# NJUVISION/PCGCv1

Measured on AMD Instinct MI355X. Metric: 64³ cubes/sec encode+decode (hyper/a6b3); bpp & D1-PSNR vs reference, higher is better.
Workload: dtype f32; 1 GPU; synthetic longdress_vox10-like cloud (seed 1300, 1024^3): 828225 points -> 205 cubes of 64^3, --mode=hyper --cube_size=64 --min_num=64, the hyper/a6b3 checkpoint trained with this repository's train_hyper step on seeded synthetic surfaces (checkpoints/hyper/a6.00b3.00, tools/train_ckpt.py; the cloud was held out), compress_hyper + decompress_hyper incl. host range coding; cubes_per_rank=205, stream_crc32=2267905730

## Files before the change

include/pcgc.h:

```cpp
#ifndef PCGC_H_
#define PCGC_H_

#include <stddef.h>
#include <stdint.h>

#ifdef __cplusplus
extern "C" {
#endif

typedef void* pcgc_stream_t;

int pcgc_version(void);
const char* pcgc_last_error(void);

int pcgc_conv3d_fwd(const float* x, const float* kernel, const float* bias, float* y,
                    int B, int D, int Cin, int Cout, int ksize, int stride,
                    int transposed, int relu, int algo, pcgc_stream_t stream);

size_t pcgc_vrn_workspace_bytes(int B, int D, int C);
int pcgc_vrn_fwd(const float* x, const float* const* params, float* out, int B, int D, int C,
                 void* workspace, size_t workspace_bytes, pcgc_stream_t stream);

enum {
  PCGC_NET_ANALYSIS = 0,
// ... 6 lines not shown
int pcgc_net_param_count(int kind);
int pcgc_net_create(int kind, const float* const* params, int n_params,
                    pcgc_stream_t stream, pcgc_net** out);
void pcgc_net_destroy(pcgc_net* net);
int pcgc_net_set_algo(pcgc_net* net, int algo);
int pcgc_rowocc(const float* x, unsigned long long* rowocc, int B, pcgc_stream_t stream);
int pcgc_net_set_skip_counter(pcgc_net* net, unsigned* device_counter);
int pcgc_net_set_profiling(pcgc_net* net, int on);
int pcgc_net_profile_report(pcgc_net* net, char* buf, size_t cap, size_t* needed);
size_t pcgc_net_workspace_bytes(const pcgc_net* net, int B, int D);
int pcgc_net_forward(const pcgc_net* net, const float* x, float* out0, float* out1,
                     int B, int D, float scale_lower_bound, void* workspace,
                     size_t workspace_bytes, pcgc_stream_t stream);


int pcgc_repro_eval(int fn, const float* x, float* y, int64_t n, pcgc_stream_t stream);

int pcgc_round_minmax(const float* x, float* q, int32_t* seg_min, int32_t* seg_max,
                      int64_t n, int64_t seg_len, pcgc_stream_t stream);
int pcgc_round_minmax_i16(const float* x, int16_t* q, int32_t* seg_min, int32_t* seg_max,
                          int64_t n, int64_t seg_len, pcgc_stream_t stream);
int pcgc_symbols_to_values(const int16_t* sym, int offset, float* out, int64_t n, pcgc_stream_t stream);
int pcgc_symbols_to_values_seg(const int16_t* sym, const float* seg_offset, float* out, int64_t n, int64_t seg_len,
                               pcgc_stream_t stream);

int pcgc_laplace_likelihood(const float* y, const float* loc, const float* scale,
                            const float* noise, float* values, float* likelihood,
                            int64_t n, float likelihood_bound, pcgc_stream_t stream);

int pcgc_laplace_cdf(const float* loc, const float* scale, const int32_t* seg_min,
                     const int32_t* seg_max, int64_t rows, int64_t seg_rows, int ncols,
                     float likelihood_bound, const float* symbols, uint16_t* cdf_lower,
                     uint32_t* lohi, pcgc_stream_t stream);

int pcgc_factorized_likelihood(const float* z, const float* params, const float* noise,
                               float* values, float* likelihood, int64_t n, int C,
                               float likelihood_bound, pcgc_stream_t stream);
int pcgc_factorized_pmf(const float* params, int C, int min_v, int max_v,
                        float likelihood_bound, float* pmf, pcgc_stream_t stream);

int pcgc_topk_threshold(const float* x, const int32_t* k_per_cube, int B, int64_t vox,
                        int use_fixed, float fixed_thres, float* thresholds,
                        uint8_t* mask, void* workspace, size_t workspace_bytes,
                        pcgc_stream_t stream);
size_t pcgc_topk_workspace_bytes(int B, int64_t vox);

int pcgc_bce_sums(const float* pred, const float* label, int64_t n, double* sums4,
                  void* workspace, size_t workspace_bytes, pcgc_stream_t stream);
size_t pcgc_bce_workspace_bytes(int64_t n);

size_t pcgc_classify_workspace_bytes(void);
int pcgc_classify_sums(const float* pred, const float* label, int64_t n, float th, double* sums3,
                       void* workspace, size_t workspace_bytes, pcgc_stream_t stream);
int pcgc_confusion_matrix(const float* pred, const float* label, int64_t n, float th, float* tp,
                          float* fp, float* fn, pcgc_stream_t stream);

size_t pcgc_focal_workspace_bytes(void);
int pcgc_focal_loss(const float* y_pred, const float* y_true, int64_t n, float gamma, float alpha, double* loss,
                    void* workspace, size_t workspace_bytes, pcgc_stream_t stream);
int pcgc_focal_loss_bwd(const float* y_pred, const float* y_true, int64_t n, float gamma, float alpha,
                        float grad_scale, float* dy_pred, pcgc_stream_t stream);

size_t pcgc_d1_workspace_bytes(int res);
int pcgc_d1_mse(const int32_t* pa, int64_t na, const int32_t* pb, int64_t nb, int res, double* out2,
                void* workspace, size_t workspace_bytes, pcgc_stream_t stream);

// ... 261 lines not shown
int pcgc_laplace_likelihood_bwd_dev(const float* values, const float* loc, const float* scale, double num, double mul,
                                    const double* count, float likelihood_bound, float* dvalues, float* dloc,
                                    float* dscale, int64_t n, pcgc_stream_t stream);
int pcgc_factorized_likelihood_bwd_dev(const float* values, const float* params, double num, double mul,
                                       const double* count, float likelihood_bound, float* dvalues, float* dparams,
                                       int64_t n, int C, void* workspace, size_t workspace_bytes, pcgc_stream_t stream);
size_t pcgc_sum_log_workspace_bytes(void);
int pcgc_sum_log(const float* p, int64_t n, double* out, void* workspace, size_t workspace_bytes,
                 pcgc_stream_t stream);
size_t pcgc_train_loss_sums_workspace_bytes(int64_t n);
int pcgc_train_loss_sums(const float* pred, const float* label, int64_t n, const float* lik_y, int64_t n_y,
                         const float* lik_z, int64_t n_z, double* sums4, double* logs2, void* workspace,
                         size_t workspace_bytes, pcgc_stream_t stream);
int pcgc_adam_step(float* param, const float* grad, float* m, float* v, int64_t n, float lr_t, float beta1,
                   float beta2, float epsilon, pcgc_stream_t stream);
int pcgc_adam_step_guarded(float* param, const float* grad, float* m, float* v, int64_t n, float lr_t, float beta1,
                           float beta2, float epsilon, const double* bce_sums4, pcgc_stream_t stream);

const char* pcgc_host_last_error(void);

int pcgc_pmf_to_quantized_cdf(const float* pmf, int64_t rows, int n, int precision, int32_t* cdf);
int pcgc_range_encode(const int16_t* data, int64_t rows, int cols, const int32_t* cdf, int n,
                      int broadcast_rows, int precision, uint8_t* out, int64_t cap, int64_t* out_len);
int pcgc_range_encode_values(const void* data, int elem_bytes, int64_t rows, int cols, int offset, const int32_t* cdf, int n,
                             int broadcast_rows, int precision, uint8_t* out, int64_t cap, int64_t* out_len);
int pcgc_range_decode(const uint8_t* str, int64_t len, int64_t rows, int cols, const int32_t* cdf,
                      int n, int broadcast_rows, int precision, int16_t* out);
int pcgc_range_decode_progress(const uint8_t* str, int64_t len, int64_t rows, int cols, const int32_t* cdf,
                               int n, int broadcast_rows, int precision, int16_t* out, int64_t* progress);

int pcgc_range_encode_lohi_batch(const uint32_t* lohi, int n_streams, int64_t sym_per_stream,
                                 int precision, uint8_t* out, int64_t cap_per_stream,
                                 int64_t* out_lens, int n_threads);
int pcgc_range_decode_u16_batch(const uint8_t* strings, const int64_t* offsets, const int64_t* lens,
                                int n_streams, int64_t sym_per_stream, const uint16_t* cdf_lower,
                                int ncols, const int32_t* n_sym, int precision, int16_t* out,
                                int n_threads);

int pcgc_partition(const int32_t* points, int64_t n, int cube_size, int min_num, int64_t* n_cubes,
                   int64_t* cube_positions, int64_t* sorted_positions, int32_t* cube_of_point);

int pcgc_parse_ply_points(const char* text, int64_t len, int32_t* out, int64_t cap, int64_t* n_points, int n_threads);

int pcgc_format_points_int(const int64_t* pts, int64_t n, char* out, int64_t cap, int64_t* out_len);

int pcgc_parse_ply_columns(const char* text, int64_t len, const int32_t* columns, int k, int64_t max_rows, double* out,
                           int64_t cap, int64_t* n_rows, int n_threads);

int pcgc_format_points_colors_int(const int64_t* pts, const uint8_t* colors, int64_t n, char* out, int64_t cap,
                                  int64_t* out_len);

int pcgc_parse_mesh(const char* text, int64_t len, int format, double* vertices, int64_t vcap, int32_t* triangles,
                    int64_t tcap, int64_t* n_vertices, int64_t* n_triangles);
int pcgc_mesh_area_cdf(const double* vertices, int64_t n_vertices, const int32_t* triangles, int64_t n_triangles, double* cdf);

uint32_t pcgc_crc32c(uint32_t crc_in, const void* data, int64_t n);

int pcgc_host_repro_eval(int fn, const float* x, float* y, int64_t n);

#ifdef __cplusplus
}
#endif
#endif
```

pcgcv1_amd/_lib.py:

```python
import ctypes
import os


_HERE = os.path.dirname(os.path.abspath(__file__))
_LIBDIR = os.path.join(_HERE, "lib")

c_int, c_i64, c_f32, c_vp, c_sz = ctypes.c_int, ctypes.c_int64, ctypes.c_float, ctypes.c_void_p, ctypes.c_size_t

HIP_API = {
    "pcgc_version": (c_int, []),
    "pcgc_last_error": (ctypes.c_char_p, []),
    "pcgc_conv3d_fwd": (c_int, [c_vp, c_vp, c_vp, c_vp, c_int, c_int, c_int, c_int, c_int, c_int, c_int, c_int, c_int, c_vp]),
    "pcgc_vrn_workspace_bytes": (c_sz, [c_int, c_int, c_int]),
    "pcgc_vrn_fwd": (c_int, [c_vp, c_vp, c_vp, c_int, c_int, c_int, c_vp, c_sz, c_vp]),
    "pcgc_net_param_count": (c_int, [c_int]),
    "pcgc_net_create": (c_int, [c_int, c_vp, c_int, c_vp, c_vp]),
    "pcgc_net_destroy": (None, [c_vp]),
    "pcgc_net_set_algo": (c_int, [c_vp, c_int]),
    "pcgc_net_set_skip_counter": (c_int, [c_vp, c_vp]),
    "pcgc_rowocc": (c_int, [c_vp, c_vp, c_int, c_vp]),
    "pcgc_net_set_profiling": (c_int, [c_vp, c_int]),
    "pcgc_net_profile_report": (c_int, [c_vp, c_vp, c_sz, c_vp]),
    "pcgc_net_workspace_bytes": (c_sz, [c_vp, c_int, c_int]),
    "pcgc_net_forward": (c_int, [c_vp, c_vp, c_vp, c_vp, c_int, c_int, c_f32, c_vp, c_sz, c_vp]),
    "pcgc_repro_eval": (c_int, [c_int, c_vp, c_vp, c_i64, c_vp]),
    "pcgc_round_minmax": (c_int, [c_vp, c_vp, c_vp, c_vp, c_i64, c_i64, c_vp]),
    "pcgc_round_minmax_i16": (c_int, [c_vp, c_vp, c_vp, c_vp, c_i64, c_i64, c_vp]),
    "pcgc_symbols_to_values": (c_int, [c_vp, c_int, c_vp, c_i64, c_vp]),
    "pcgc_symbols_to_values_seg": (c_int, [c_vp, c_vp, c_vp, c_i64, c_i64, c_vp]),
    "pcgc_laplace_likelihood": (c_int, [c_vp, c_vp, c_vp, c_vp, c_vp, c_vp, c_i64, c_f32, c_vp]),
    "pcgc_laplace_cdf": (c_int, [c_vp, c_vp, c_vp, c_vp, c_i64, c_i64, c_int, c_f32, c_vp, c_vp, c_vp, c_vp]),
    "pcgc_factorized_likelihood": (c_int, [c_vp, c_vp, c_vp, c_vp, c_vp, c_i64, c_int, c_f32, c_vp]),
    "pcgc_factorized_pmf": (c_int, [c_vp, c_int, c_int, c_int, c_f32, c_vp, c_vp]),
    "pcgc_topk_threshold": (c_int, [c_vp, c_vp, c_int, c_i64, c_int, c_f32, c_vp, c_vp, c_vp, c_sz, c_vp]),
    "pcgc_topk_workspace_bytes": (c_sz, [c_int, c_i64]),
    "pcgc_bce_sums": (c_int, [c_vp, c_vp, c_i64, c_vp, c_vp, c_sz, c_vp]),
    "pcgc_bce_workspace_bytes": (c_sz, [c_i64]),
    "pcgc_classify_workspace_bytes": (c_sz, []),
    "pcgc_classify_sums": (c_int, [c_vp, c_vp, c_i64, c_f32, c_vp, c_vp, c_sz, c_vp]),
    "pcgc_confusion_matrix": (c_int, [c_vp, c_vp, c_i64, c_f32, c_vp, c_vp, c_vp, c_vp]),
    "pcgc_focal_workspace_bytes": (c_sz, []),
    "pcgc_focal_loss": (c_int, [c_vp, c_vp, c_i64, c_f32, c_f32, c_vp, c_vp, c_sz, c_vp]),
    "pcgc_focal_loss_bwd": (c_int, [c_vp, c_vp, c_i64, c_f32, c_f32, c_f32, c_vp, c_vp]),
    "pcgc_voxelize": (c_int, [c_vp, c_i64, c_int, c_vp, c_int, c_vp]),
    "pcgc_voxelize_points": (c_int, [c_vp, c_vp, c_i64, c_int, c_int, c_int, c_vp, c_vp]),
    "pcgc_pointnums_count": (c_int, [c_vp, c_vp, c_vp, c_int, c_int, c_vp, c_vp, c_vp, c_vp]),
    "pcgc_pointnums_curves_workspace_bytes": (c_sz, [c_i64, c_i64]),
    "pcgc_pointnums_curves": (c_int, [c_vp, c_vp, c_vp, c_int, c_int, c_vp, c_vp, c_vp, c_i64, c_i64, c_vp, c_int, c_vp, c_int,
                                      c_vp, c_vp, c_vp, c_vp, c_sz, c_vp]),
    "pcgc_pointnums_normals_workspace_bytes": (c_sz, [c_i64]),
    "pcgc_pointnums_normals": (c_int, [c_vp, c_vp, c_i64, c_vp, c_i64, c_vp, c_vp, c_sz, c_vp]),
    "pcgc_pointnums_curves_d2_workspace_bytes": (c_sz, [c_i64, c_i64]),
    "pcgc_pointnums_curves_d2": (c_int, [c_vp, c_vp, c_vp, c_vp, c_int, c_int, c_vp, c_vp, c_vp, c_i64, c_i64, c_vp, c_int, c_vp,
                                         c_int, c_vp, c_vp, c_vp, c_vp, c_sz, c_vp]),
    "pcgc_pointnums_sweep_workspace_bytes": (c_sz, [c_int, c_int]),
    "pcgc_pointnums_sweep": (c_int, [c_vp, c_vp, c_vp, c_vp, c_int, c_int, c_vp, c_int, c_vp, c_vp, c_vp, c_sz, c_vp]),
    "pcgc_mesh_sample": (c_int, [c_vp, c_i64, c_vp, c_i64, c_vp, c_i64, ctypes.c_uint64, c_vp, c_vp, c_vp]),
    "pcgc_mesh_voxelize_workspace_bytes": (c_sz, [c_int]),
    "pcgc_mesh_voxelize": (c_int, [c_vp, c_i64, c_int, c_vp, c_i64, c_vp, c_vp, c_sz, c_vp]),
    "pcgc_normals_table_size": (c_int, [ctypes.c_double]),
    "pcgc_normals_workspace_bytes": (c_sz, [c_int, c_i64, ctypes.c_double]),
    "pcgc_estimate_normals": (c_int, [c_vp, c_i64, c_int, ctypes.c_double, c_int, c_vp, c_vp, c_vp, c_vp, c_sz, c_vp]),
    "pcgc_ingest_bounds": (c_int, [c_vp, c_i64, c_vp, c_vp, c_vp]),
    "pcgc_ingest_quantize": (c_int, [c_vp, c_i64, c_vp, ctypes.c_double, c_int, c_vp, c_vp, c_vp]),
# ... 94 lines not shown
    "pcgc_train_conv_fwd": (c_int, [c_vp, c_int, c_vp, c_vp, c_vp, c_int, c_int, c_int, c_vp]),
    "pcgc_train_conv_bwd_data": (c_int, [c_vp, c_int, c_vp, c_vp, c_vp, c_vp, c_int, c_int, c_vp]),
    "pcgc_train_conv_bwd_weight": (c_int, [c_vp, c_int, c_vp, c_vp, c_int, c_int, c_vp]),
    "pcgc_train_conv_bwd_weight_pair": (c_int, [c_vp, c_int, c_int, c_vp, c_vp, c_vp, c_int, c_int, c_vp]),
    "pcgc_train_conv_fwd_pair": (c_int, [c_vp, c_int, c_int, c_vp, c_vp, c_vp, c_vp, c_vp, c_vp, c_int, c_int, c_int, c_int, c_vp]),
    "pcgc_train_conv_bwd_data_pair": (c_int, [c_vp, c_int, c_int, c_vp, c_vp, c_vp, c_vp, c_vp, c_vp, c_int, c_int, c_vp]),
    "pcgc_train_conv_bwd_data_chain": (c_int, [c_vp, c_int, c_int, c_vp, c_vp, c_vp, c_vp, c_int, c_int, c_vp]),
    "pcgc_train_conv_fwd_merge": (c_int, [c_vp, c_int, c_vp, c_vp, c_vp, c_int, c_vp, c_vp, c_vp, c_int, c_int, c_int, c_vp]),
    "pcgc_train_plan_finish_weights": (c_int, [c_vp, c_vp]),
    "pcgc_train_plan_defer_small": (c_int, [c_vp, c_int]),
    "pcgc_abs_max": (c_int, [c_vp, c_f32, c_vp, c_vp, c_i64, c_vp]),
    "pcgc_laplace_likelihood_bwd": (c_int, [c_vp, c_vp, c_vp, c_f32, c_f32, c_vp, c_vp, c_vp, c_i64, c_vp]),
    "pcgc_factorized_bwd_workspace_bytes": (c_sz, [c_int]),
    "pcgc_factorized_likelihood_bwd": (c_int, [c_vp, c_vp, c_f32, c_f32, c_vp, c_vp, c_i64, c_int, c_vp, c_sz, c_vp]),
    "pcgc_bce_bwd": (c_int, [c_vp, c_vp, c_f32, c_f32, c_vp, c_i64, c_vp]),
    "pcgc_bce_bwd_dev": (c_int, [c_vp, c_vp, c_vp, ctypes.c_double, ctypes.c_double, c_vp, c_i64, c_vp]),
    "pcgc_laplace_likelihood_bwd_dev": (c_int, [c_vp, c_vp, c_vp, ctypes.c_double, ctypes.c_double, c_vp, c_f32, c_vp, c_vp, c_vp, c_i64, c_vp]),
    "pcgc_factorized_likelihood_bwd_dev": (c_int, [c_vp, c_vp, ctypes.c_double, ctypes.c_double, c_vp, c_f32, c_vp, c_vp, c_i64, c_int, c_vp, c_sz, c_vp]),
    "pcgc_sum_log_workspace_bytes": (c_sz, []),
    "pcgc_sum_log": (c_int, [c_vp, c_i64, c_vp, c_vp, c_sz, c_vp]),
    "pcgc_train_loss_sums_workspace_bytes": (c_sz, [c_i64]),
    "pcgc_train_loss_sums": (c_int, [c_vp, c_vp, c_i64, c_vp, c_i64, c_vp, c_i64, c_vp, c_vp, c_vp, c_sz, c_vp]),
    "pcgc_adam_step": (c_int, [c_vp, c_vp, c_vp, c_vp, c_i64, c_f32, c_f32, c_f32, c_f32, c_vp]),
    "pcgc_adam_step_guarded": (c_int, [c_vp, c_vp, c_vp, c_vp, c_i64, c_f32, c_f32, c_f32, c_f32, c_vp, c_vp]),
}
HOST_API = {
    "pcgc_host_last_error": (ctypes.c_char_p, []),
    "pcgc_pmf_to_quantized_cdf": (c_int, [c_vp, c_i64, c_int, c_int, c_vp]),
    "pcgc_range_encode": (c_int, [c_vp, c_i64, c_int, c_vp, c_int, c_int, c_int, c_vp, c_i64, c_vp]),
    "pcgc_range_encode_values": (c_int, [c_vp, c_int, c_i64, c_int, c_int, c_vp, c_int, c_int, c_int, c_vp, c_i64, c_vp]),
    "pcgc_range_decode": (c_int, [c_vp, c_i64, c_i64, c_int, c_vp, c_int, c_int, c_int, c_vp]),
    "pcgc_range_decode_progress": (c_int, [c_vp, c_i64, c_i64, c_int, c_vp, c_int, c_int, c_int, c_vp, c_vp]),
    "pcgc_range_encode_lohi_batch": (c_int, [c_vp, c_int, c_i64, c_int, c_vp, c_i64, c_vp, c_int]),
    "pcgc_range_decode_u16_batch": (c_int, [c_vp, c_vp, c_vp, c_int, c_i64, c_vp, c_int, c_vp, c_int, c_vp, c_int]),
    "pcgc_partition": (c_int, [c_vp, c_i64, c_int, c_int, c_vp, c_vp, c_vp, c_vp]),
    "pcgc_crc32c": (ctypes.c_uint32, [ctypes.c_uint32, c_vp, c_i64]),
    "pcgc_host_repro_eval": (c_int, [c_int, c_vp, c_vp, c_i64]),
    "pcgc_format_points_int": (c_int, [c_vp, c_i64, c_vp, c_i64, c_vp]),
    "pcgc_parse_ply_points": (c_int, [c_vp, c_i64, c_vp, c_i64, c_vp, c_int]),
    "pcgc_parse_ply_columns": (c_int, [c_vp, c_i64, c_vp, c_int, c_i64, c_vp, c_i64, c_vp, c_int]),
    "pcgc_format_points_colors_int": (c_int, [c_vp, c_vp, c_i64, c_vp, c_i64, c_vp]),
    "pcgc_parse_mesh": (c_int, [c_vp, c_i64, c_int, c_vp, c_i64, c_vp, c_i64, c_vp, c_vp]),
    "pcgc_mesh_area_cdf": (c_int, [c_vp, c_i64, c_vp, c_i64, c_vp]),
}

_hip = None
_host = None


class PcgcError(RuntimeError):
    pass


def _load(name, api):
    path = os.path.join(_LIBDIR, name)
    if not os.path.exists(path):
        raise PcgcError("%s is not built: run `python -m pcgcv1_amd.build` (hipcc --offload-arch=gfx950). "
                        "There is no CPU fallback for the hot path." % path)
    lib = ctypes.CDLL(path)
    for fn, (res, args) in api.items():
        f = getattr(lib, fn)
        f.restype = res
        f.argtypes = args
    return lib


# ... 128 lines not shown
```

pcgcv1_amd/csrc/entropy.hip:

```cpp
#include <climits>
#include <cmath>
#include <map>
#include <mutex>
#include <vector>

#include "common.h"
#include "repro_math.h"

namespace pcgc {

__global__ void fill_minmax_kernel(int32_t* mn, int32_t* mx, int n) {
  const int i = blockIdx.x * 256 + threadIdx.x;
  if (i < n) { mn[i] = INT_MAX; mx[i] = INT_MIN; }
}

template <typename Q>
__global__ void __launch_bounds__(256) round_minmax_kernel(const float* x, Q* q, int32_t* seg_min, int32_t* seg_max,
                                                           int64_t seg_len, int blocks_per_seg) {
  const int seg = blockIdx.x / blocks_per_seg, part = blockIdx.x % blocks_per_seg;
  const int64_t base = (int64_t)seg * seg_len;
  int lo = INT_MAX, hi = INT_MIN;
  for (int64_t i = (int64_t)part * 256 + threadIdx.x; i < seg_len; i += (int64_t)blocks_per_seg * 256) {
    const float r = rintf(x[base + i]);
    const int v = (int)r;
// ... 199 lines not shown
            D -= F;
          }
        }
      }
    }
    while (D > 0) {
      int h = 0, ba = age[0];
      double bk = key[0];
#pragma unroll
      for (int k = 1; k < MAXN; ++k)
        if (k < N && (key[k] > bk || (key[k] == bk && age[k] < ba))) { h = k; bk = key[k]; ba = age[k]; }
#pragma unroll
      for (int k = 0; k < MAXN; ++k)
        if (k == h) {
          v[k] += sd;
          key[k] = ckey((double)mass[k], v[k]);
          age[k] = stamp;
        }
      ++stamp;
      --D;
    }
  }
  int sym = -1;
  if (symbols) sym = (int)symbols[row] - mn;
  int acc = 0;
  uint32_t lh = 0;
#pragma unroll
  for (int k = 0; k < MAXN; ++k) {
    if (k < ncols && cdf_lower) cdf_lower[row * ncols + k] = (uint16_t)(k < N ? acc : 0xFFFF);
    if (k == sym) lh = (uint32_t)acc | ((uint32_t)(acc + v[k] - 1) << 16);
    acc += v[k];
  }
  if (lohi) lohi[row] = lh;
}

struct FactorizedParams {
  float m0[3], b0[3], f0[3];
  float m1[9], b1[3], f1[3];
  float m2[9], b2[3], f2[3];
  float m3[3], b3[1], f3[1];
};

__device__ __forceinline__ float softplusf(float x) { return repro::softplusf_(x); }
__device__ __forceinline__ float tanhr(float x) { return repro::tanhf_(x); }

__device__ void load_factorized(const float* p, int C, int c, FactorizedParams& P) {
  const float* m0 = p;              const float* b0 = m0 + C * 3; const float* f0 = b0 + C * 3;
  const float* m1 = f0 + C * 3;     const float* b1 = m1 + C * 9; const float* f1 = b1 + C * 3;
  const float* m2 = f1 + C * 3;     const float* b2 = m2 + C * 9; const float* f2 = b2 + C * 3;
  const float* m3 = f2 + C * 3;     const float* b3 = m3 + C * 3; const float* f3 = b3 + C;
  for (int i = 0; i < 3; ++i) { P.m0[i] = softplusf(m0[c * 3 + i]); P.b0[i] = b0[c * 3 + i]; P.f0[i] = tanhr(f0[c * 3 + i]); }
  for (int i = 0; i < 9; ++i) { P.m1[i] = softplusf(m1[c * 9 + i]); P.m2[i] = softplusf(m2[c * 9 + i]); }
  for (int i = 0; i < 3; ++i) {
    P.b1[i] = b1[c * 3 + i]; P.f1[i] = tanhr(f1[c * 3 + i]);
    P.b2[i] = b2[c * 3 + i]; P.f2[i] = tanhr(f2[c * 3 + i]);
    P.m3[i] = softplusf(m3[c * 3 + i]);
  }
  P.b3[0] = b3[c]; P.f3[0] = tanhr(f3[c]);
}

__device__ __forceinline__ float logits_cumulative(const FactorizedParams& P, float x) {
  float a[3], t[3];
#pragma unroll
  for (int i = 0; i < 3; ++i) { a[i] = P.m0[i] * x + P.b0[i]; a[i] = a[i] + P.f0[i] * tanhr(a[i]); }
#pragma unroll
  for (int i = 0; i < 3; ++i) {
// ... 146 lines not shown
  if (blocks > 8192) blocks = 8192;
  hipLaunchKernelGGL(laplace_likelihood_kernel, dim3(blocks), dim3(256), 0, (hipStream_t)stream, y, loc, scale, noise,
                     values, likelihood, n, likelihood_bound);
  return launch_ok("laplace_likelihood_kernel");
}

int pcgc_laplace_cdf(const float* loc, const float* scale, const int32_t* seg_min, const int32_t* seg_max, int64_t rows,
                     int64_t seg_rows, int ncols, float likelihood_bound, const float* symbols, uint16_t* cdf_lower,
                     uint32_t* lohi, pcgc_stream_t stream) {
  if (rows == 0) return 0;
  PCGC_REQUIRE(loc && scale && seg_min && seg_max && seg_rows > 0 && rows % seg_rows == 0, "pcgc_laplace_cdf: bad arguments");
  PCGC_REQUIRE(ncols >= 1 && ncols <= 32, "pcgc_laplace_cdf: ncols=%d outside [1,32] (the container stores |min|,|max| <= 15)", ncols);
  PCGC_REQUIRE(!lohi || symbols, "pcgc_laplace_cdf: lohi needs symbols");
  if (rows == 0) return 0;
  dim3 grid((unsigned)((rows + 255) / 256)), block(256);
  hipStream_t s = (hipStream_t)stream;
  const double* lg = nullptr;
  { int rc = get_log2_table(&lg); if (rc) return rc; }
  if (ncols <= 4)
    hipLaunchKernelGGL(laplace_cdf_kernel<4>, grid, block, 0, s, loc, scale, seg_min, seg_max, rows, seg_rows, ncols,
                       likelihood_bound, symbols, cdf_lower, lohi, lg);
  else if (ncols <= 8)
    hipLaunchKernelGGL(laplace_cdf_kernel<8>, grid, block, 0, s, loc, scale, seg_min, seg_max, rows, seg_rows, ncols,
                       likelihood_bound, symbols, cdf_lower, lohi, lg);
  else if (ncols <= 16)
    hipLaunchKernelGGL(laplace_cdf_kernel<16>, grid, block, 0, s, loc, scale, seg_min, seg_max, rows, seg_rows, ncols,
                       likelihood_bound, symbols, cdf_lower, lohi, lg);
  else
    hipLaunchKernelGGL(laplace_cdf_kernel<32>, grid, block, 0, s, loc, scale, seg_min, seg_max, rows, seg_rows, ncols,
                       likelihood_bound, symbols, cdf_lower, lohi, lg);
  return launch_ok("laplace_cdf_kernel");
}

int pcgc_factorized_likelihood(const float* z, const float* params, const float* noise, float* values, float* likelihood,
                               int64_t n, int C, float likelihood_bound, pcgc_stream_t stream) {
  if (n == 0) return 0;
  PCGC_REQUIRE(z && params && C > 0 && C <= kMaxFactorizedC && n % C == 0, "pcgc_factorized_likelihood: bad arguments (C=%d)", C);
  if (n == 0) return 0;
  int blocks = (int)((n + 255) / 256);
  if (blocks > 4096) blocks = 4096;
  hipLaunchKernelGGL(factorized_likelihood_kernel, dim3(blocks), dim3(256), 0, (hipStream_t)stream, z, params, noise,
                     values, likelihood, n, C, likelihood_bound);
  return launch_ok("factorized_likelihood_kernel");
}

int pcgc_factorized_pmf(const float* params, int C, int min_v, int max_v, float likelihood_bound, float* pmf,
                        pcgc_stream_t stream) {
  PCGC_REQUIRE(params && pmf && C > 0 && max_v >= min_v, "pcgc_factorized_pmf: bad arguments");
  const int N = max_v - min_v + 1;
  hipLaunchKernelGGL(factorized_pmf_kernel, dim3((C * N + 63) / 64), dim3(64), 0, (hipStream_t)stream, params, C, min_v, N,
                     likelihood_bound, pmf);
  return launch_ok("factorized_pmf_kernel");
}

}
```

pcgcv1_amd/csrc/host.cpp:

```cpp
#include <algorithm>
#include <atomic>
#include <cmath>
#include <cstdarg>
#include <cstdint>
#include <cstdio>
#include <cstdlib>
#include <chrono>
#include <cstring>
#include <limits>
#include <condition_variable>
#include <mutex>
#include <pthread.h>
#include <numeric>
#include <string>
#include <thread>
#include <unordered_map>
#include <vector>

#include "../../include/pcgc.h"
#include "repro_math.h"

namespace {

thread_local char g_err[512] = "";
// ... 362 lines not shown
  if (elem_bytes == 1)
    return range_encode_values(static_cast<const int8_t*>(data), rows, cols, offset, cdf, n, broadcast_rows, precision, out, cap, out_len);
  return range_encode_values(static_cast<const int16_t*>(data), rows, cols, offset, cdf, n, broadcast_rows, precision, out, cap, out_len);
}

int pcgc_range_decode(const uint8_t* str, int64_t len, int64_t rows, int cols, const int32_t* cdf, int n,
                      int broadcast_rows, int precision, int16_t* out) {
  return range_decode_impl(str, len, rows, cols, cdf, n, broadcast_rows, precision, out, nullptr);
}

int pcgc_range_decode_progress(const uint8_t* str, int64_t len, int64_t rows, int cols, const int32_t* cdf, int n,
                               int broadcast_rows, int precision, int16_t* out, int64_t* progress) {
  if (!progress) { set_error("pcgc_range_decode_progress: progress is NULL"); return -1; }
  return range_decode_impl(str, len, rows, cols, cdf, n, broadcast_rows, precision, out, progress);
}

int pcgc_range_encode_lohi_batch(const uint32_t* lohi, int n_streams, int64_t sym_per_stream, int precision,
                                 uint8_t* out, int64_t cap_per_stream, int64_t* out_lens, int n_threads) {
  if (n_streams < 0 || (n_streams > 0 && (!lohi || !out || !out_lens))) { set_error("pcgc_range_encode_lohi_batch: NULL argument"); return -1; }
  std::atomic<int> bad(0);
  parallel_for(n_streams, n_threads, [&](int sidx) {
    Sink sink{out + int64_t(sidx) * cap_per_stream, cap_per_stream};
    RangeEncoder enc;
    const uint32_t* p = lohi + int64_t(sidx) * sym_per_stream;
    for (int64_t i = 0; i < sym_per_stream; ++i) {
      const uint32_t w = p[i];
      enc.encode(w & 0xFFFFu, (w >> 16) + 1u, precision, sink);
    }
    enc.finalize(sink);
    out_lens[sidx] = sink.len;
    if (sink.len > cap_per_stream) bad.store(1);
  });
  if (bad.load()) { set_error("pcgc_range_encode_lohi_batch: a stream exceeded cap_per_stream=%lld", (long long)cap_per_stream); return -2; }
  return 0;
}

int pcgc_range_decode_u16_batch(const uint8_t* strings, const int64_t* offsets, const int64_t* lens, int n_streams,
                                int64_t sym_per_stream, const uint16_t* cdf_lower, int ncols, const int32_t* n_sym,
                                int precision, int16_t* out, int n_threads) {
  if (n_streams < 0 || (n_streams > 0 && (!offsets || !lens || !cdf_lower || !n_sym || !out))) { set_error("pcgc_range_decode_u16_batch: NULL argument"); return -1; }
  std::atomic<int> bad(0);
  const uint32_t top = 1u << precision;
  parallel_for(n_streams, n_threads, [&](int sidx) {
    RangeDecoder dec(strings + offsets[sidx], lens[sidx]);
    const int n = n_sym[sidx];
    if (n < 1 || n > ncols) { bad.store(1); return; }
    const uint16_t* rows = cdf_lower + int64_t(sidx) * sym_per_stream * ncols;
    int16_t* o = out + int64_t(sidx) * sym_per_stream;
    for (int64_t i = 0; i < sym_per_stream; ++i) {
      const uint16_t* row = rows + i * ncols;
      const int s = dec.decode(n, precision, [row, n, top](int k) { return k >= n ? top : uint32_t(row[k]); });
      if (s < 0) { bad.store(2); return; }
      o[i] = int16_t(s);
    }
  });
  if (bad.load()) { set_error("pcgc_range_decode_u16_batch: %s", bad.load() == 1 ? "n_sym outside [1,ncols]" : "corrupt stream"); return -3; }
  return 0;
}

int pcgc_partition(const int32_t* points, int64_t n, int cube_size, int min_num, int64_t* n_cubes,
                   int64_t* cube_positions, int64_t* sorted_positions, int32_t* cube_of_point) {
  if (!n_cubes || (n > 0 && !points) || cube_size <= 0) { set_error("pcgc_partition: bad arguments"); return -1; }
  auto fdiv = [cube_size](int32_t v) -> int64_t { return v >= 0 ? v / cube_size : -((-(int64_t)v + cube_size - 1) / cube_size); };
  struct Key { int64_t x, y, z; bool operator==(const Key& o) const { return x == o.x && y == o.y && z == o.z; } };
  struct H { size_t operator()(const Key& k) const { return size_t(k.x * 73856093LL ^ k.y * 19349663LL ^ k.z * 83492791LL); } };
  std::vector<Key> keys;
// ... 612 lines not shown
```

pcgcv1_amd/models/conditional_entropy_model.py:

```python
import numpy as np
import torch

from .. import _lib

_MAX_SYMBOLS = 32
_SLICES = int(__import__("os").environ.get("PCGC_SLICES", "2"))


_SLICE_ALIGN = int(__import__("os").environ.get("PCGC_SLICE_ALIGN", "8"))


def _slices(B, n):
    n = max(1, min(n, B // 32))
    base, rem = divmod(B, n)
    out, lo = [], 0
    for i in range(n):
        hi = lo + base + (1 if i < rem else 0)
        if i + 1 < n and _SLICE_ALIGN > 1:
            hi = min(B, -(-hi // _SLICE_ALIGN) * _SLICE_ALIGN)
        hi = B if i + 1 == n else hi
        out.append((lo, hi))
        lo = hi
    return [s_ for s_ in out if s_[1] > s_[0]]


def decode_slices(B, first=None, n=None, row_bytes=0, tail=0):
    first = (_FIRST_SLICE if _FIRST_SLICE >= 0 else 24) if first is None else first
    n = max(_DEC_SLICES, B // 100) if n is None else n
    if first <= 0 or B < first + 32:
        return _slices(B, n)
    rest = B - first
    if tail > 0 and n == 1 and rest >= 2 * tail + 16:
        cut = ((B - tail) // 8) * 8
        return [(0, first), (first, cut), (cut, B)]
    return [(0, first)] + [(first + lo, first + hi) for lo, hi in _slices(rest, n)]


_DEC_SLICES = int(__import__("os").environ.get("PCGC_DEC_SLICES", "1"))
_FIRST_SLICE = int(__import__("os").environ.get("PCGC_FIRST_SLICE", "-1"))


class SymmetricConditional(object):
    def __init__(self, likelihood_bound=1e-9, range_coder_precision=16):
        self._likelihood_bound = float(likelihood_bound)
        self._range_coder_precision = int(range_coder_precision)
        if self._range_coder_precision != 16:
            raise NotImplementedError("the device CDF kernel emits 16-bit CDFs (the reference's only setting)")
        self._pinned = {}
        self._guards = {}

    @staticmethod
    def _dev(t):
        dev = _lib.require_gpu()
        if not torch.is_tensor(t):
            t = torch.from_numpy(np.ascontiguousarray(t, np.float32))
        return t.to(dev, torch.float32).contiguous()

    def _side_stream(self, role, cur):
        return _lib.side_stream(role, cur)

    def _guard(self, what, cur):
        ev = self._guards.pop((what, int(cur.cuda_stream)), None)
        if ev is not None:
            ev.synchronize()

    def _pin(self, key, shape, dtype):
        key = (key, int(torch.cuda.current_stream().cuda_stream))
        n = int(np.prod(shape))
        buf = self._pinned.get(key)
        if buf is None or buf.numel() < n or buf.dtype != dtype:
            buf = torch.empty(max(n, 1), dtype=dtype, pin_memory=True)
            self._pinned[key] = buf
        return buf[:n].view(*shape)

    def __call__(self, inputs, loc, scale, training, noise=None):
        x, loc, scale = self._dev(inputs), self._dev(loc), self._dev(scale)
        if training and noise is None:
            noise = torch.rand_like(x) - 0.5
        if noise is not None:
            noise = self._dev(noise)
        values, lik = torch.empty_like(x), torch.empty_like(x)
        _lib.check(_lib.hip().pcgc_laplace_likelihood(_lib.dptr(x), _lib.dptr(loc), _lib.dptr(scale),
                                                      _lib.dptr(noise) if training else None, _lib.dptr(values),
                                                      _lib.dptr(lik), x.numel(), self._likelihood_bound, _lib.stream()),
                   "pcgc_laplace_likelihood")
        return values, lik

    def quantize_minmax(self, ys, n_seg):
        q = torch.empty_like(ys)
        mn = torch.empty(n_seg, dtype=torch.int32, device=ys.device)
        mx = torch.empty(n_seg, dtype=torch.int32, device=ys.device)
        _lib.check(_lib.hip().pcgc_round_minmax(_lib.dptr(ys), _lib.dptr(q), _lib.dptr(mn), _lib.dptr(mx), ys.numel(),
                                                ys.numel() // n_seg, _lib.stream()), "pcgc_round_minmax")
        return q, mn, mx

    def _check_range(self, mn, mx):
        n = int((mx - mn).max()) + 1
        if n > _MAX_SYMBOLS:
            raise ValueError("symbol range of %d values exceeds %d (the container stores |min|,|max| <= 15, "
                             "inout_bitstream.py:95-96)" % (n, _MAX_SYMBOLS))
        assert int((mx - mn).min()) >= 1
        return n

    @staticmethod
    def _widen(mn, mx):
        mn, mx = np.minimum(mn, 0), np.maximum(mx, 0)
        same = mx == mn
        if same.any():
            mx = np.where(same & (mx < 15), mx + 1, mx)
            mn = np.where(same & (mx == mn), mn - 1, mn)
        return mn.astype(np.int32), mx.astype(np.int32)

    def start_ranges(self, ys):
        ys = self._dev(ys)
        B = int(ys.shape[0])
        if B == 0:
            return None
        y_hat, mn_d, mx_d = self.quantize_minmax(ys, B)
        host_mm = self._pin("minmax", (2, B), torch.int32)
        host_mm[0].copy_(mn_d, non_blocking=True)
        host_mm[1].copy_(mx_d, non_blocking=True)
        ev = torch.cuda.Event()
        ev.record()
        return y_hat, mn_d, mx_d, host_mm, ev

    def compress_cubes(self, ys, locs, scales, n_threads=None, n_slices=_SLICES, ranges=None):
        ys, locs, scales = self._dev(ys), self._dev(locs), self._dev(scales)
        B = int(ys.shape[0])
        if B == 0:
            return [], np.zeros(0, np.int32), np.zeros(0, np.int32)
        rows = ys.numel()
        seg = rows // B
        lib, host = _lib.hip(), _lib.host()
        y_hat, mn_d, mx_d, host_mm, ev = ranges if ranges is not None else self.start_ranges(ys)
        ev.synchronize()
        _lib.mark("enc ranges on the host")
        mn0, mx0 = host_mm[0].numpy().copy(), host_mm[1].numpy().copy()
        mn, mx = self._widen(mn0, mx0)
        if not (np.array_equal(mn, mn0) and np.array_equal(mx, mx0)):
            mn_d, mx_d = torch.from_numpy(mn).to(ys.device), torch.from_numpy(mx).to(ys.device)
        ncols = self._check_range(mn, mx)
        lohi = torch.empty(rows, dtype=torch.int32, device=ys.device)
        host_lohi = self._pin("lohi", (rows,), torch.int32)
        yf, lf, sf = y_hat.reshape(-1), locs.reshape(-1), scales.reshape(-1)
        events = []
        for lo, hi in _slices(B, n_slices):
            a, b = lo * seg, hi * seg
            _lib.check(lib.pcgc_laplace_cdf(_lib.dptr(lf[a:b]), _lib.dptr(sf[a:b]), _lib.dptr(mn_d[lo:hi]), _lib.dptr(mx_d[lo:hi]),
                                            b - a, seg, ncols, self._likelihood_bound, _lib.dptr(yf[a:b]), None,
                                            _lib.dptr(lohi[a:b]), _lib.stream()), "pcgc_laplace_cdf")
            host_lohi[a:b].copy_(lohi[a:b], non_blocking=True)
            ev = torch.cuda.Event()
            ev.record()
            events.append((lo, hi, ev))
        cap = seg * 2 + 1024
        out = self._pin("enc_out", (B, cap), torch.uint8).numpy()
        lens = np.zeros(B, np.int64)
        nt = n_threads or _lib.host_threads()
        _lib.mark("enc cdf slices queued")
        for lo, hi, ev in events:
            ev.synchronize()
            _lib.mark("enc slice [%d:%d] on the host" % (lo, hi))
            _lib.check_host(host.pcgc_range_encode_lohi_batch(host_lohi[lo * seg:].data_ptr(), hi - lo, seg,
                                                              self._range_coder_precision, _lib.nptr(out[lo:hi]), cap,
                                                              _lib.nptr(lens[lo:hi]), nt), "pcgc_range_encode_lohi_batch")
        strings = [out[i, :lens[i]].tobytes() for i in range(B)]
        return strings, mn.astype(np.int32), mx.astype(np.int32)

    def compress(self, inputs, loc, scale):
        x = self._dev(inputs)
        s, mn, mx = self.compress_cubes(x.reshape((1,) + tuple(x.shape)), self._dev(loc).reshape((1,) + tuple(x.shape)),
                                        self._dev(scale).reshape((1,) + tuple(x.shape)), n_threads=1)
        return s[0], int(mn[0]), int(mx[0])

    def decompress_slices(self, strings, locs, scales, min_vs, max_vs, datashape, n_threads=None, n_slices=_SLICES, slices=None):
        lazy = callable(locs)
        if not lazy:
            locs, scales = self._dev(locs), self._dev(scales)
        B = len(strings)
        datashape = tuple(int(s) for s in datashape)
        per_cube = int(np.prod(datashape))
        cube_shape = datashape[1:] if datashape[0] == 1 else datashape
        if B == 0:
            return
        dev = _lib.require_gpu()
        assert lazy or (locs.numel() == B * per_cube and scales.numel() == B * per_cube)
        lib, host = _lib.hip(), _lib.host()
        mn = np.ascontiguousarray(min_vs, np.int32).reshape(B)
        mx = np.ascontiguousarray(max_vs, np.int32).reshape(B)
        ncols = self._check_range(mn, mx)
        rows = B * per_cube
        cur = torch.cuda.current_stream()
        es, us = self._side_stream("entropy", cur), self._side_stream("upload", cur)
        start = torch.cuda.Event()
        start.record(cur)
        es.wait_event(start)
        us.wait_event(start)
        todo = list(slices) if slices else _slices(B, n_slices)
# ... 96 lines not shown
```

Baseline: 5176 cubes/s.

## Pack lohi words on device as default-bitmask plus exceptions before host encode

Adds a GPU kernel that compresses each stream's per-symbol lohi words into a 64-bit 'equals default symbol' bitmask per 64 symbols plus a bounded exception list, and a host range encoder that consumes this packed form. The goal is to shrink the device-to-host copy of the full int32 lohi array ahead of range coding. If a stream has more than K exceptions it falls back to copying the full lohi array, and it remembers that overflow per stream so later calls skip packing until a background check shows the packed form would fit again. The cost is an extra kernel launch and added bookkeeping, and mostly-default streams are also encoded faster through a fast path.

```diff
diff --git a/include/pcgc.h b/include/pcgc.h
--- a/include/pcgc.h
+++ b/include/pcgc.h
@@ -62,6 +62,10 @@
                      const int32_t* seg_max, int64_t rows, int64_t seg_rows, int ncols,
                      float likelihood_bound, const float* symbols, uint16_t* cdf_lower,
                      uint32_t* lohi, pcgc_stream_t stream);
+
+int pcgc_lohi_pack(const uint32_t* lohi, const uint32_t* default_word, int n_streams,
+                   int64_t sym_per_stream, int K, uint64_t* codes, uint32_t* exceptions,
+                   int32_t* counts, pcgc_stream_t stream);
 
 int pcgc_factorized_likelihood(const float* z, const float* params, const float* noise,
                                float* values, float* likelihood, int64_t n, int C,
@@ -389,6 +393,10 @@
 int pcgc_range_encode_lohi_batch(const uint32_t* lohi, int n_streams, int64_t sym_per_stream,
                                  int precision, uint8_t* out, int64_t cap_per_stream,
                                  int64_t* out_lens, int n_threads);
+int pcgc_range_encode_packed_batch(const uint64_t* codes, const uint32_t* exceptions, const int32_t* counts,
+                                   const uint32_t* default_word, int K, int n_streams,
+                                   int64_t sym_per_stream, int precision, uint8_t* out,
+                                   int64_t cap_per_stream, int64_t* out_lens, int n_threads);
 int pcgc_range_decode_u16_batch(const uint8_t* strings, const int64_t* offsets, const int64_t* lens,
                                 int n_streams, int64_t sym_per_stream, const uint16_t* cdf_lower,
                                 int ncols, const int32_t* n_sym, int precision, int16_t* out,
diff --git a/pcgcv1_amd/_lib.py b/pcgcv1_amd/_lib.py
--- a/pcgcv1_amd/_lib.py
+++ b/pcgcv1_amd/_lib.py
@@ -30,6 +30,7 @@
     "pcgc_symbols_to_values_seg": (c_int, [c_vp, c_vp, c_vp, c_i64, c_i64, c_vp]),
     "pcgc_laplace_likelihood": (c_int, [c_vp, c_vp, c_vp, c_vp, c_vp, c_vp, c_i64, c_f32, c_vp]),
     "pcgc_laplace_cdf": (c_int, [c_vp, c_vp, c_vp, c_vp, c_i64, c_i64, c_int, c_f32, c_vp, c_vp, c_vp, c_vp]),
+    "pcgc_lohi_pack": (c_int, [c_vp, c_vp, c_int, c_i64, c_int, c_vp, c_vp, c_vp, c_vp]),
     "pcgc_factorized_likelihood": (c_int, [c_vp, c_vp, c_vp, c_vp, c_vp, c_i64, c_int, c_f32, c_vp]),
     "pcgc_factorized_pmf": (c_int, [c_vp, c_int, c_int, c_int, c_f32, c_vp, c_vp]),
     "pcgc_topk_threshold": (c_int, [c_vp, c_vp, c_int, c_i64, c_int, c_f32, c_vp, c_vp, c_vp, c_sz, c_vp]),
@@ -190,6 +191,7 @@
     "pcgc_range_decode": (c_int, [c_vp, c_i64, c_i64, c_int, c_vp, c_int, c_int, c_int, c_vp]),
     "pcgc_range_decode_progress": (c_int, [c_vp, c_i64, c_i64, c_int, c_vp, c_int, c_int, c_int, c_vp, c_vp]),
     "pcgc_range_encode_lohi_batch": (c_int, [c_vp, c_int, c_i64, c_int, c_vp, c_i64, c_vp, c_int]),
+    "pcgc_range_encode_packed_batch": (c_int, [c_vp, c_vp, c_vp, c_vp, c_int, c_int, c_i64, c_int, c_vp, c_i64, c_vp, c_int]),
     "pcgc_range_decode_u16_batch": (c_int, [c_vp, c_vp, c_vp, c_int, c_i64, c_vp, c_int, c_vp, c_int, c_vp, c_int]),
     "pcgc_partition": (c_int, [c_vp, c_i64, c_int, c_int, c_vp, c_vp, c_vp, c_vp]),
     "pcgc_crc32c": (ctypes.c_uint32, [ctypes.c_uint32, c_vp, c_i64]),
diff --git a/pcgcv1_amd/csrc/entropy.hip b/pcgcv1_amd/csrc/entropy.hip
--- a/pcgcv1_amd/csrc/entropy.hip
+++ b/pcgcv1_amd/csrc/entropy.hip
@@ -255,6 +255,49 @@
     acc += v[k];
   }
   if (lohi) lohi[row] = lh;
+}
+
+constexpr int kPackWaves = 16;
+
+__global__ void __launch_bounds__(kPackWaves * 64) lohi_pack_kernel(const uint32_t* __restrict__ lohi,
+                                                                    const uint32_t* __restrict__ default_word, int64_t sym_per_stream,
+                                                                    int K, uint64_t* __restrict__ codes, uint32_t* __restrict__ exc,
+                                                                    int32_t* __restrict__ counts) {
+  __shared__ int wave_count[kPackWaves];
+  const int64_t s = blockIdx.x;
+  const int wave = threadIdx.x >> 6, lane = threadIdx.x & 63;
+  const int64_t units = sym_per_stream / 64;
+  const int64_t u0 = units * wave / kPackWaves, u1 = units * (wave + 1) / kPackWaves;
+  const uint32_t* p = lohi + s * sym_per_stream;
+  const uint32_t dw = default_word[s];
+  int cnt = 0;
+#pragma unroll 8
+  for (int64_t u = u0; u < u1; ++u) {
+    const unsigned long long same = __ballot(p[u * 64 + lane] == dw);
+    if (lane == 0) codes[s * units + u] = same;
+    cnt += 64 - __popcll(same);
+  }
+  if (lane == 0) wave_count[wave] = cnt;
+  __syncthreads();
+  int off = 0, total = 0;
+#pragma unroll
+  for (int i = 0; i < kPackWaves; ++i) {
+    off += i < wave ? wave_count[i] : 0;
+    total += wave_count[i];
+  }
+  if (threadIdx.x == 0) counts[s] = total;
+  if (cnt == 0 || off >= K) return;
+  const unsigned long long below = (1ull << lane) - 1ull;
+#pragma unroll 8
+  for (int64_t u = u0; u < u1; ++u) {
+    const uint32_t w = p[u * 64 + lane];
+    const unsigned long long other = __ballot(w != dw);
+    if (w != dw) {
+      const int idx = off + __popcll(other & below);
+      if (idx < K) exc[s * K + idx] = w;
+    }
+    off += __popcll(other);
+  }
 }
 
 struct FactorizedParams {
@@ -467,6 +510,17 @@
   return launch_ok("laplace_cdf_kernel");
 }
 
+int pcgc_lohi_pack(const uint32_t* lohi, const uint32_t* default_word, int n_streams, int64_t sym_per_stream, int K,
+                   uint64_t* codes, uint32_t* exceptions, int32_t* counts, pcgc_stream_t stream) {
+  if (n_streams == 0) return 0;
+  PCGC_REQUIRE(lohi && default_word && codes && exceptions && counts && n_streams > 0 && K >= 0, "pcgc_lohi_pack: bad arguments");
+  PCGC_REQUIRE(sym_per_stream > 0 && sym_per_stream % 64 == 0, "pcgc_lohi_pack: sym_per_stream=%lld must be a multiple of 64",
+               (long long)sym_per_stream);
+  hipLaunchKernelGGL(lohi_pack_kernel, dim3((unsigned)n_streams), dim3(kPackWaves * 64), 0, (hipStream_t)stream, lohi, default_word,
+                     sym_per_stream, K, codes, exceptions, counts);
+  return launch_ok("lohi_pack_kernel");
+}
+
 int pcgc_factorized_likelihood(const float* z, const float* params, const float* noise, float* values, float* likelihood,
                                int64_t n, int C, float likelihood_bound, pcgc_stream_t stream) {
   if (n == 0) return 0;
diff --git a/pcgcv1_amd/csrc/host.cpp b/pcgcv1_amd/csrc/host.cpp
--- a/pcgcv1_amd/csrc/host.cpp
+++ b/pcgcv1_amd/csrc/host.cpp
@@ -418,6 +418,58 @@
     if (sink.len > cap_per_stream) bad.store(1);
   });
   if (bad.load()) { set_error("pcgc_range_encode_lohi_batch: a stream exceeded cap_per_stream=%lld", (long long)cap_per_stream); return -2; }
+  return 0;
+}
+
+int pcgc_range_encode_packed_batch(const uint64_t* codes, const uint32_t* exceptions, const int32_t* counts,
+                                   const uint32_t* default_word, int K, int n_streams, int64_t sym_per_stream, int precision,
+                                   uint8_t* out, int64_t cap_per_stream, int64_t* out_lens, int n_threads) {
+  if (n_streams < 0 || (n_streams > 0 && (!codes || !exceptions || !counts || !default_word || !out || !out_lens))) {
+    set_error("pcgc_range_encode_packed_batch: NULL argument");
+    return -1;
+  }
+  if (K < 0 || sym_per_stream < 0 || sym_per_stream % 64 != 0) {
+    set_error("pcgc_range_encode_packed_batch: K=%d, sym_per_stream=%lld (must be a multiple of 64)", K, (long long)sym_per_stream);
+    return -1;
+  }
+  for (int sidx = 0; sidx < n_streams; ++sidx)
+    if (counts[sidx] < 0 || counts[sidx] > K) {
+      set_error("pcgc_range_encode_packed_batch: stream %d has %d exceptions, the list holds K=%d", sidx, counts[sidx], K);
+      return counts[sidx] < 0 ? -1 : -4;
+    }
+  const int64_t units = sym_per_stream / 64;
+  std::atomic<int> bad(0);
+  parallel_for(n_streams, n_threads, [&](int sidx) {
+    Sink sink{out + int64_t(sidx) * cap_per_stream, cap_per_stream};
+    RangeEncoder enc;
+    const uint64_t* code = codes + int64_t(sidx) * units;
+    const uint32_t* ex = exceptions + int64_t(sidx) * K;
+    const uint32_t* ex_end = ex + counts[sidx];
+    const uint32_t dw = default_word[sidx];
+    const uint32_t dlo = dw & 0xFFFFu, dhi = (dw >> 16) + 1u;
+    for (int64_t u = 0; u < units; ++u) {
+      const uint64_t same = code[u];
+      if (same == ~uint64_t(0)) {
+        for (int i = 0; i < 64; ++i) enc.encode(dlo, dhi, precision, sink);
+        continue;
+      }
+      for (int i = 0; i < 64; ++i) {
+        if ((same >> i) & 1u) {
+          enc.encode(dlo, dhi, precision, sink);
+        } else {
+          if (ex == ex_end) { bad.fetch_or(2); return; }
+          const uint32_t w = *ex++;
+          enc.encode(w & 0xFFFFu, (w >> 16) + 1u, precision, sink);
+        }
+      }
+    }
+    if (ex != ex_end) { bad.fetch_or(2); return; }
+    enc.finalize(sink);
+    out_lens[sidx] = sink.len;
+    if (sink.len > cap_per_stream) bad.fetch_or(1);
+  });
+  if (bad.load() & 2) { set_error("pcgc_range_encode_packed_batch: codes and counts disagree"); return -1; }
+  if (bad.load()) { set_error("pcgc_range_encode_packed_batch: a stream exceeded cap_per_stream=%lld", (long long)cap_per_stream); return -2; }
   return 0;
 }
 
diff --git a/pcgcv1_amd/models/conditional_entropy_model.py b/pcgcv1_amd/models/conditional_entropy_model.py
--- a/pcgcv1_amd/models/conditional_entropy_model.py
+++ b/pcgcv1_amd/models/conditional_entropy_model.py
@@ -1,9 +1,12 @@
+import os
+
 import numpy as np
 import torch
 
 from .. import _lib
 
 _MAX_SYMBOLS = 32
+_PACK_K = 2048
 _SLICES = int(__import__("os").environ.get("PCGC_SLICES", "2"))
 
 
@@ -48,6 +51,7 @@
             raise NotImplementedError("the device CDF kernel emits 16-bit CDFs (the reference's only setting)")
         self._pinned = {}
         self._guards = {}
+        self._pack_overflowed = {}
 
     @staticmethod
     def _dev(t):
@@ -110,6 +114,10 @@
             mx = np.where(same & (mx < 15), mx + 1, mx)
             mn = np.where(same & (mx == mn), mn - 1, mn)
         return mn.astype(np.int32), mx.astype(np.int32)
+
+    @staticmethod
+    def _default_words(mn, mx):
+        return ((-mn).astype(np.int64) | ((65535 - mx.astype(np.int64)) << 16)).astype(np.uint32)
 
     def start_ranges(self, ys):
         ys = self._dev(ys)
@@ -141,18 +149,49 @@
             mn_d, mx_d = torch.from_numpy(mn).to(ys.device), torch.from_numpy(mx).to(ys.device)
         ncols = self._check_range(mn, mx)
         lohi = torch.empty(rows, dtype=torch.int32, device=ys.device)
-        host_lohi = self._pin("lohi", (rows,), torch.int32)
         yf, lf, sf = y_hat.reshape(-1), locs.reshape(-1), scales.reshape(-1)
-        events = []
+        key = int(torch.cuda.current_stream().cuda_stream)
+        pack = seg % 64 == 0 and os.environ.get("PCGC_LOHI_PACK", "1") != "0"
+        packed = pack and not self._pack_overflowed.get(key, False)
+        if pack:
+            K, units = _PACK_K, seg // 64
+            rec8 = units + K // 2 + 1
+
+            def parts(buf, lo, hi):
+                n, r = hi - lo, buf[lo * rec8:hi * rec8]
+                return r[:n * units], r[n * units:n * (units + K // 2)].view(torch.int32), r[n * (units + K // 2):].view(torch.int32)[:n]
+
+            def queue_pack(lo, hi):
+                codes, exc, cnt = parts(pack_d, lo, hi)
+                _lib.check(lib.pcgc_lohi_pack(_lib.dptr(lohi[lo * seg:hi * seg]), _lib.dptr(dw_d[lo:hi]), hi - lo, seg, K, _lib.dptr(codes),
+                                              _lib.dptr(exc), _lib.dptr(cnt), _lib.stream()), "pcgc_lohi_pack")
+        host_lohi = None if packed else self._pin("lohi", (rows,), torch.int32)
+        events, dw_d = [], None
         for lo, hi in _slices(B, n_slices):
             a, b = lo * seg, hi * seg
             _lib.check(lib.pcgc_laplace_cdf(_lib.dptr(lf[a:b]), _lib.dptr(sf[a:b]), _lib.dptr(mn_d[lo:hi]), _lib.dptr(mx_d[lo:hi]),
                                             b - a, seg, ncols, self._likelihood_bound, _lib.dptr(yf[a:b]), None,
                                             _lib.dptr(lohi[a:b]), _lib.stream()), "pcgc_laplace_cdf")
-            host_lohi[a:b].copy_(lohi[a:b], non_blocking=True)
+            if pack and dw_d is None:
+                dw_host = self._pin("pack_dw", (B,), torch.int32)
+                dw_host.numpy()[:] = self._default_words(mn, mx).view(np.int32)
+                dw_d = dw_host.to(ys.device, non_blocking=True)
+                pack_d = torch.empty(B * rec8, dtype=torch.int64, device=ys.device)
+                host_pack = self._pin("pack", (B * rec8,), torch.int64)
+            if packed:
+                queue_pack(lo, hi)
+                host_pack[lo * rec8:hi * rec8].copy_(pack_d[lo * rec8:hi * rec8], non_blocking=True)
+            else:
+                host_lohi[a:b].copy_(lohi[a:b], non_blocking=True)
             ev = torch.cuda.Event()
             ev.record()
             events.append((lo, hi, ev))
+        hint = None
+        if pack and not packed:
+            queue_pack(0, B)
+            parts(host_pack, 0, B)[2].copy_(parts(pack_d, 0, B)[2], non_blocking=True)
+            hint = torch.cuda.Event()
+            hint.record()
         cap = seg * 2 + 1024
         out = self._pin("enc_out", (B, cap), torch.uint8).numpy()
         lens = np.zeros(B, np.int64)
@@ -161,9 +200,27 @@
         for lo, hi, ev in events:
             ev.synchronize()
             _lib.mark("enc slice [%d:%d] on the host" % (lo, hi))
-            _lib.check_host(host.pcgc_range_encode_lohi_batch(host_lohi[lo * seg:].data_ptr(), hi - lo, seg,
+            a, b = lo * seg, hi * seg
+            if packed:
+                codes, exc, cnt = parts(host_pack, lo, hi)
+                if int(cnt.max()) <= K:
+                    _lib.check_host(host.pcgc_range_encode_packed_batch(
+                        codes.data_ptr(), exc.data_ptr(), cnt.data_ptr(), dw_host[lo:].data_ptr(), K, hi - lo, seg,
+                        self._range_coder_precision, _lib.nptr(out[lo:hi]), cap, _lib.nptr(lens[lo:hi]), nt),
+                        "pcgc_range_encode_packed_batch")
+                    continue
+                self._pack_overflowed[key] = True
+                if host_lohi is None:
+                    host_lohi = self._pin("lohi", (rows,), torch.int32)
+                host_lohi[a:b].copy_(lohi[a:b])
+                _lib.mark("enc slice [%d:%d] overflowed its pack" % (lo, hi))
+            _lib.check_host(host.pcgc_range_encode_lohi_batch(host_lohi[a:].data_ptr(), hi - lo, seg,
                                                               self._range_coder_precision, _lib.nptr(out[lo:hi]), cap,
                                                               _lib.nptr(lens[lo:hi]), nt), "pcgc_range_encode_lohi_batch")
+        if hint is not None:
+            hint.synchronize()
+            if int(parts(host_pack, 0, B)[2].max()) <= K:
+                self._pack_overflowed.pop(key, None)
         strings = [out[i, :lens[i]].tobytes() for i in range(B)]
         return strings, mn.astype(np.int32), mx.astype(np.int32)
 
```

After: 5215 cubes/s (median of 3 runs). Within noise of the previous version (+0.8%).
